# ivanalberico/End-To-End-Self-Supervised-SLAM

Measured on AMD Instinct MI355X. Metric: online refinement steps/sec @640x480, seq_len=60, higher is better.
Workload: dtype f32

## Files before the change

### end-to-end-self-supervised-slam_amd/csrc/conv.hip

```cpp
#include <cassert>
#include <type_traits>

#include "e2e_common.h"

typedef float f4v __attribute__((ext_vector_type(4)));
typedef float f16v __attribute__((ext_vector_type(16)));

#define CBK 16

enum { ACT_NONE = 0, ACT_RELU = 1, ACT_ELU = 2, ACT_DISP = 3 };

struct ConvArgs {
    const float* src0;
    const float* src1;
    const float* w;
    const float* scale;
    const float* shift;
    const float* res;
    float* out;
    int B, Hs, Ws;
    int Cin, C1, up;
    int Hd, Wd;
    int Ncols, ldw;
    int KH, KW, stride, pad, pad_mode;
// ... 1750 lines not shown
#pragma unroll
        for (int j = 0; j < PH; ++j) *(f4v*)&patch[(j * PW * 4 + tid) * 4] = preg[j];
        if (tid < PH * 8) *(f4v*)&patch[((epy * PW + epx) * 4 + pq) * 4] = preg[PH];
    };
    f4v acc[NA];
#pragma unroll
    for (int t = 0; t < NA; ++t) acc[t] = (f4v){0.f, 0.f, 0.f, 0.f};
    const float one = (l16 == 0) ? 1.f : 0.f;
    const float* bp = patch + (wave * PW + kq) * 16 + l16;
    auto sweep = [&](unsigned zn) {
        float bv[9];
#pragma unroll
        for (int t = 0; t < 9; ++t) bv[t] = bp[((t / 3) * PW + (t % 3)) * 16];
#pragma unroll
        for (int ks = 0; ks < TW / 4; ++ks) {
            float bn[9];
#pragma unroll
            for (int t = 0; t < 9; ++t) bn[t] = ks + 1 < TW / 4 ? bp[((t / 3) * PW + (t % 3)) * 16 + (ks + 1) * 64] : 0.f;
#pragma unroll
            for (int t = 0; t < 9; ++t)
#pragma unroll
                for (int mt = 0; mt < MT; ++mt) acc[mt * 10 + t] = __builtin_amdgcn_mfma_f32_16x16x4f32(areg[ks][mt], bv[t], acc[mt * 10 + t], 0, 0, 0);
            if constexpr (BIAS) {
#pragma unroll
                for (int mt = 0; mt < MT; ++mt) acc[mt * 10 + 9] = __builtin_amdgcn_mfma_f32_16x16x4f32(areg[ks][mt], one, acc[mt * 10 + 9], 0, 0, 0);
            }
#pragma unroll
            for (int mt = 0; mt < MT; ++mt)
                areg[ks][mt] = __builtin_bit_cast(float, __builtin_amdgcn_raw_buffer_load_b32(rz, zn + (unsigned)(ks * 4 * CO + mt * 16) * 4u, 0, 0));
#pragma unroll
            for (int t = 0; t < 9; ++t) bv[t] = bn[t];
            __builtin_amdgcn_sched_barrier(0);
        }
    };
    if (ntl > 0) {
        load_dz((unsigned)(tx0 * TW * CO) * 4u + zl);
        load_patch(tx0 * TW);
        store_patch();
    }
    __syncthreads();
    for (int tx = 0; tx < ntl; ++tx) {
        const bool more = tx + 1 < ntl;
        const int xn = (tx0 + tx + 1) * TW;
        const unsigned zn = more ? (unsigned)(xn * CO) * 4u + zl : OOB;
        if (more) load_patch(xn);
        sweep(zn);
        __syncthreads();
        if (more) {
            store_patch();
            __syncthreads();
        }
    }
    float* red = smem;
    const int64_t sid = ((int64_t)b * gridDim.y + blockIdx.y) * a.nxg + blockIdx.x;
    float* slab = a.slabs + sid * CO * a.npad;
    const int kconv = 9 * a.Cin, cg0 = hf * 16;
#pragma unroll
    for (int mt = 0; mt < MT; ++mt) {
        if (mt > 0) __syncthreads();
        if (wave >= 2) {
#pragma unroll
            for (int t = 0; t < 10; ++t)
#pragma unroll
                for (int i = 0; i < 4; ++i) red[((wave - 2) * 40 + t * 4 + i) * 64 + lane] = acc[mt * 10 + t][i];
        }
        __syncthreads();
        if (wave < 2) {
#pragma unroll
            for (int t = 0; t < 10; ++t)
#pragma unroll
                for (int i = 0; i < 4; ++i) acc[mt * 10 + t][i] += red[(wave * 40 + t * 4 + i) * 64 + lane];
        }
        __syncthreads();
        if (wave == 1) {
#pragma unroll
            for (int t = 0; t < 10; ++t)
#pragma unroll
                for (int i = 0; i < 4; ++i) red[(t * 4 + i) * 64 + lane] = acc[mt * 10 + t][i];
        }
        __syncthreads();
        if (wave == 0) {
#pragma unroll
            for (int t = 0; t < 10; ++t)
#pragma unroll
                for (int i = 0; i < 4; ++i) {
                    const float v = acc[mt * 10 + t][i] + red[(t * 4 + i) * 64 + lane];
                    const int co = mt * 16 + 4 * kq + i;
                    if (t < 9) slab[co * a.npad + t * a.Cin + cg0 + l16] = v;
                    else if (BIAS && l16 == 0) slab[co * a.npad + kconv] = v;
                }
        }
    }
}

template <int MT>
__global__ __launch_bounds__(256) __attribute__((amdgpu_waves_per_eu(MT == 1 ? 4 : 2))) void k_wgrad3x3_thin_regs(ThinWgradArgs a) {
    __shared__ float smem[6 * 66 * 16];
    if (a.has_bias && blockIdx.z % (a.Cin >> 4) == 0) wgrad3x3_thin_regs_body<MT, true>(a, smem);
    else wgrad3x3_thin_regs_body<MT, false>(a, smem);
}

struct StemWgradArgs {
    const float* dz;
    const float* src;
    float* slabs;
    int B, Hs, Ws, Hd, Wd, tiles_x, nxg;
    float in_sub, in_mul;
};

__global__ __launch_bounds__(256) void k_wgrad7x7_stem(StemWgradArgs a) {
    constexpr int TH = 4, TW = 32, PH = 2 * TH + 6, PW = 2 * TW + 5, ROW = 208, NPAD = 148;
    __shared__ float patch[PH * ROW];
    __shared__ float dzs[TH * TW * 64];
    const int tid = threadIdx.x, lane = tid & 63, wave = tid >> 6, l16 = lane & 15, kq = lane >> 4;
    const int y0 = blockIdx.y * TH, b = blockIdx.z;
    int offn[10];
#pragma unroll
    for (int nt = 0; nt < 10; ++nt) {
        const int k = 16 * nt + l16;
        offn[nt] = k + (k / 21) * (ROW - 21) + 48 * kq;
    }
    f4v acc[10];
#pragma unroll
    for (int nt = 0; nt < 10; ++nt) acc[nt] = (f4v){0.f, 0.f, 0.f, 0.f};
    const float* sb = a.src + (int64_t)b * a.Hs * a.Ws * 3;
    const float* zb = a.dz + (int64_t)b * a.Hd * a.Wd * 64;
    for (int tx = 0; tx < a.tiles_x; ++tx) {
        const int x0 = (blockIdx.x * a.tiles_x + tx) * TW;
        if (x0 >= a.Wd) break;
        __syncthreads();
        for (int idx = tid; idx < PH * ROW; idx += 256) {
            const int py = idx / ROW, e = idx - py * ROW;
            const int Y = 2 * y0 - 3 + py, X = 2 * x0 - 3 + e / 3;
            const bool ok = e < 3 * PW && Y >= 0 && Y < a.Hs && X >= 0 && X < a.Ws;
            patch[idx] = ok ? (sb[((int64_t)Y * a.Ws + X) * 3 + (e - (e / 3) * 3)] - a.in_sub) * a.in_mul : 0.f;
        }
        for (int idx = tid; idx < TH * TW * 16; idx += 256) {
            const int q = idx & 15, pix = idx >> 4;
            const int r = pix / TW, x = pix - r * TW;
            const bool ok = y0 + r < a.Hd && x0 + x < a.Wd;
            *(f4v*)&dzs[pix * 64 + q * 4] = ok ? *(const f4v*)(zb + ((int64_t)(y0 + r) * a.Wd + x0 + x) * 64 + q * 4) : (f4v){0.f, 0.f, 0.f, 0.f};
        }
        __syncthreads();
#pragma unroll 1
        for (int r = 0; r < TH; ++r) {
            const float* ap = dzs + (r * TW + 8 * kq) * 64 + 16 * wave + l16;
            const float* bp = patch + 2 * r * ROW;
#pragma unroll 2
            for (int ks = 0; ks < TW / 4; ++ks) {
                const float av = ap[ks * 64];
#pragma unroll
                for (int nt = 0; nt < 10; ++nt) acc[nt] = __builtin_amdgcn_mfma_f32_16x16x4f32(av, bp[offn[nt] + ks * 6], acc[nt], 0, 0, 0);
            }
        }
    }
    float* slab = a.slabs + (((int64_t)b * gridDim.y + blockIdx.y) * a.nxg + blockIdx.x) * 64 * NPAD;
#pragma unroll
    for (int nt = 0; nt < 10; ++nt)
#pragma unroll
        for (int i = 0; i < 4; ++i) {
            const int n = 16 * nt + l16;
            if (n < 147) slab[(16 * wave + 4 * kq + i) * NPAD + n] = acc[nt][i];
        }
}

struct TapWgradArgs {
    const float* dz;
    const float* src0;
    const float* src1;
    float* slabs;
    int B, H, W, Cin, C1, up, Cout, reflect, has_bias, Mpad, Npad;
    int ptx, pty;
    int nchunks, cps;
};

#define TAP_NT 192
template <bool BIAS>
__global__ __launch_bounds__(TAP_NT) void k_wgrad3x3_taps(TapWgradArgs a) {
    __shared__ float dzs[64 * 32];
    __shared__ float xs[100 * 32];
    const int tid = threadIdx.x, lane = tid & 63, wave = tid >> 6, kh_ = lane >> 5, l32 = lane & 31;
    const int ci0 = blockIdx.x * 32, co0 = blockIdx.y * 32;
    const bool first = ci0 < a.C1;
    const int sh = first ? (a.up >> 1) : 0, Cs = first ? a.C1 : a.Cin - a.C1, cs0 = first ? ci0 : ci0 - a.C1;
    const int Hs = a.H >> sh, Ws = a.W >> sh;
    const float* sbase = first ? a.src0 : a.src1;
    const int c_begin = blockIdx.z * a.cps, c_end = min(c_begin + a.cps, a.nchunks);
    const bool want_bias = BIAS && blockIdx.x == 0 && wave == 0;
    f16v acc[3], accb;
#pragma unroll
    for (int t = 0; t < 3; ++t)
#pragma unroll
        for (int r = 0; r < 16; ++r) acc[t][r] = 0.f;
#pragma unroll
    for (int r = 0; r < 16; ++r) accb[r] = 0.f;
    const float one = (l32 == 0) ? 1.f : 0.f;
    f4v rz[3], rx[5];
    auto load_chunk = [&](int g) {
        const int b = g / (a.pty * a.ptx), rem = g - b * (a.pty * a.ptx), py = rem / a.ptx, px = rem - py * a.ptx;
        const int y0 = py * 8, x0 = px * 8;
        const float* zb = a.dz + (int64_t)b * a.H * a.W * a.Cout + co0;
        const float* sb = sbase + (int64_t)b * Hs * Ws * Cs + cs0;
#pragma unroll
        for (int i = 0; i < 3; ++i) {
            const int f = tid + TAP_NT * i, pix = f >> 3, q = f & 7, y = y0 + (pix >> 3), x = x0 + (pix & 7);
            const bool ok = f < 512 && y < a.H && x < a.W;
            rz[i] = ok ? *(const f4v*)(zb + ((int64_t)y * a.W + x) * a.Cout + q * 4) : (f4v){0.f, 0.f, 0.f, 0.f};
        }
#pragma unroll
        for (int i = 0; i < 5; ++i) {
            const int f = tid + TAP_NT * i;
            f4v v = {0.f, 0.f, 0.f, 0.f};
            if (f < 800) {
                const int pix = f >> 3, q = f & 7;
                int y = y0 - 1 + pix / 10, x = x0 - 1 + pix % 10;
                bool ok = true;
                if (a.reflect) {
                    y = min(max(reflect1(y, a.H), 0), a.H - 1);
                    x = min(max(reflect1(x, a.W), 0), a.W - 1);
                } else {
                    ok = y >= 0 && y < a.H && x >= 0 && x < a.W;
                }
                if (ok) v = *(const f4v*)(sb + ((int64_t)(y >> sh) * Ws + (x >> sh)) * Cs + q * 4);
            }
            rx[i] = v;
        }
    };
    auto store_chunk = [&]() {
#pragma unroll
        for (int i = 0; i < 3; ++i) {
            const int f = tid + TAP_NT * i;
            if (f < 512) *(f4v*)&dzs[f * 4] = rz[i];
        }
#pragma unroll
        for (int i = 0; i < 5; ++i) {
            const int f = tid + TAP_NT * i;
            if (f < 800) *(f4v*)&xs[f * 4] = rx[i];
        }
    };
    if (c_begin < c_end) load_chunk(c_begin);
    const float* ap = dzs + kh_ * 32 + l32;
    const float* bp = xs + (kh_ + wave * 10) * 32 + l32;
    for (int c = c_begin; c < c_end; ++c) {
        __syncthreads();
        store_chunk();
        __syncthreads();
        if (c + 1 < c_end) load_chunk(c + 1);
        constexpr int QB = 4, NQ = 32 / QB;
        float av[2][QB], bv[2][QB][3];
        auto read_q = [&](int set, int qt) {
#pragma unroll
            for (int j = 0; j < QB; ++j) {
                const int ks = QB * qt + j, q0 = (ks >> 2) * 10 + 2 * (ks & 3);
                av[set][j] = ap[2 * ks * 32];
#pragma unroll
                for (int t = 0; t < 3; ++t) bv[set][j][t] = bp[(q0 + t) * 32];
            }
        };
        auto pin_q = [&](int set) {
#pragma unroll
            for (int j = 0; j < QB; ++j) {
                asm volatile("" : "+v"(av[set][j]));
#pragma unroll
                for (int t = 0; t < 3; ++t) asm volatile("" : "+v"(bv[set][j][t]));
            }
        };
        read_q(0, 0);
#pragma unroll
        for (int qt = 0; qt < NQ; ++qt) {
            if (qt + 1 < NQ) read_q((qt + 1) & 1, qt + 1);
            __builtin_amdgcn_sched_barrier(0);
            pin_q(qt & 1);
            __builtin_amdgcn_sched_barrier(0);
#pragma unroll
            for (int j = 0; j < QB; ++j) {
#pragma unroll
                for (int t = 0; t < 3; ++t) acc[t] = __builtin_amdgcn_mfma_f32_32x32x2f32(av[qt & 1][j], bv[qt & 1][j][t], acc[t], 0, 0, 0);
                if (BIAS && want_bias) accb = __builtin_amdgcn_mfma_f32_32x32x2f32(av[qt & 1][j], one, accb, 0, 0, 0);
            }
            __builtin_amdgcn_sched_barrier(0);
        }
    }
    float* slab = a.slabs + (int64_t)blockIdx.z * a.Mpad * a.Npad;
#pragma unroll
    for (int t = 0; t < 3; ++t)
#pragma unroll
        for (int r = 0; r < 16; ++r) {
            const int m = co0 + (r & 3) + 8 * (r >> 2) + 4 * kh_;
            slab[(int64_t)m * a.Npad + (wave * 3 + t) * a.Cin + ci0 + l32] = acc[t][r];
        }
    if (BIAS && want_bias && l32 == 0) {
#pragma unroll
        for (int r = 0; r < 16; ++r) slab[(int64_t)(co0 + (r & 3) + 8 * (r >> 2) + 4 * kh_) * a.Npad + 9 * a.Cin] = accb[r];
    }
}

template <int ZL, int NW>
__device__ __forceinline__ void wgrad_reduce_group(const float* __restrict__ slabs, int S, int Mpad, int Npad, int Cout, int Cin, int KH, int KW, int has_bias,
                                                   float* __restrict__ dw, float* __restrict__ dbias, int accumulate, const float* __restrict__ scale,
                                                   int64_t base, int e, int w, f4v (*part)[64]) {
    const int Kconv = KH * KW * Cin, Ng = Kconv + (has_bias ? 1 : 0);
    const int nq = (Ng + 3) / 4;
    const int64_t totalq = (int64_t)Cout * nq;
    const int64_t slab_q = (int64_t)Mpad * Npad / 4;
    const f4v zero = {0.f, 0.f, 0.f, 0.f};
    const int64_t q = base + e;
// ... 1036 lines not shown
#define HEAD_PARTS 2048
int e2e_head_fwd(const float* x, const float* w, const float* bias, float* y, int B, int H, int W, int Cin, int act, void* stream) {
    E2E_REQUIRE(x && w && y && B > 0 && H >= 2 && W >= 2 && Cin == HC, E2E_ERR_ARG, "e2e_head_fwd: bad argument (the head takes %d channels)", HC);
    hipLaunchKernelGGL(k_head_fwd, dim3(egrid((int64_t)B * H * W * 4)), dim3(256), 0, (hipStream_t)stream, x, w, bias, y, B, H, W, act);
    E2E_LAUNCH_CHECK("e2e_head_fwd");
    return E2E_OK;
}
int64_t e2e_head_workspace_floats(void) { return (int64_t)HEAD_PARTS * (9 * HC + 1); }
int e2e_head_bwd_act(const float* dz, const float* x, const float* w, float* dx, float* dw, float* dbias, float* workspace, int B, int H,
                     int W, int Cin, int in_act, void* stream) {
    E2E_REQUIRE(dz && x && w && workspace && B > 0 && H >= 2 && W >= 2 && Cin == HC && in_act >= 0 && in_act <= 2, E2E_ERR_ARG, "e2e_head_bwd: bad argument");
    E2E_REQUIRE((int64_t)B * H * W * HC < (1ll << 31), E2E_ERR_ARG, "e2e_head_bwd: activation too large for 32-bit element offsets");
    hipStream_t st = (hipStream_t)stream;
    const char* ev = getenv("E2E_HEAD_BWD_FUSED");
    if (dx && dw && !(ev && ev[0] == '0')) {
        hipLaunchKernelGGL(k_head_bwd_fused, dim3(HEAD_PARTS), dim3(256), 0, st, dz, x, w, dx, workspace, B, H, W, in_act);
        hipLaunchKernelGGL(k_head_wreduce, dim3(9 * HC + 1), dim3(256), 0, st, workspace, HEAD_PARTS, dw, dbias);
        E2E_LAUNCH_CHECK("e2e_head_bwd");
        return E2E_OK;
    }
    if (dx) hipLaunchKernelGGL(k_head_bwd_data, dim3(egrid((int64_t)B * H * W * 4)), dim3(256), 0, st, dz, w, dx, B, H, W, x, in_act);
    if (dw) {
        hipLaunchKernelGGL(k_head_bwd_weight, dim3(HEAD_PARTS), dim3(256), 0, st, dz, x, workspace, B, H, W);
        hipLaunchKernelGGL(k_head_wreduce, dim3(9 * HC + 1), dim3(256), 0, st, workspace, HEAD_PARTS, dw, dbias);
    }
    E2E_LAUNCH_CHECK("e2e_head_bwd");
    return E2E_OK;
}

int e2e_head_bwd(const float* dz, const float* x, const float* w, float* dx, float* dw, float* dbias, float* workspace, int B, int H,
                 int W, int Cin, void* stream) {
    return e2e_head_bwd_act(dz, x, w, dx, dw, dbias, workspace, B, H, W, Cin, 0, stream);
}

enum WgradPath { WP_STEM, WP_THIN, WP_TAPS, WP_GEMM16, WP_GEMM_LEAN, WP_GEMM, WP_COUNT };
struct WgradPlan { WgradPath path; bool open; int64_t S; int Mpad, Npad, tm, tn, nxg, ny, tiles_x, ptx, pty, nchunks, cps; };
#define TAP_TARGET 640
static WgradPlan wgrad_plan(WgradPath path, const ConvGeom& g, int has_bias, bool tuned, int wg_target) {
    const int B = g.B, Ho = g.Ho, Wo = g.Wo, Cin = g.Cin, Cout = g.Cout, KH = g.KH, KW = g.KW;
    WgradPlan p{path};
    if (path == WP_STEM) {
        if (tuned || !(KH == 7 && KW == 7 && Cin == 3 && Cout == 64)) return p;
        p.nxg = ((Wo + 31) / 32 + 1) / 2; p.ny = (Ho + 3) / 4;
        p.S = (int64_t)B * p.ny * p.nxg; p.Mpad = 64; p.Npad = 148;
    } else if (path == WP_THIN) {
        if (tuned || !(KH == 3 && KW == 3 && ((Cout == 16 && (Cin == 16 || Cin == 32)) || (Cout == 32 && Cin == 96)))) return p;
        const int txt = (Wo + 63) / 64;
        p.ny = (Ho + 3) / 4;
        const int64_t total = (int64_t)B * p.ny * txt * (Cin / 16);
        p.tiles_x = 1;
        while (total / p.tiles_x > 1400 && p.tiles_x < txt) ++p.tiles_x;
        p.nxg = (txt + p.tiles_x - 1) / p.tiles_x;
        p.S = (int64_t)B * p.ny * p.nxg; p.Mpad = Cout; p.Npad = (9 * Cin + (has_bias ? 1 : 0) + 3) / 4 * 4;
    } else if (path == WP_TAPS) {
        if (tuned || !(KH == 3 && KW == 3 && Cin % 32 == 0 && Cout % 32 == 0)) return p;
        p.ptx = (Wo + 7) / 8; p.pty = (Ho + 7) / 8;
        p.nchunks = B * p.ptx * p.pty;
        const int tiles = (Cin / 32) * (Cout / 32);
        int S = (TAP_TARGET + tiles - 1) / tiles;
        if (S > p.nchunks) S = p.nchunks;
        if (S < 1) S = 1;
        p.cps = (p.nchunks + S - 1) / S;
        p.S = (p.nchunks + p.cps - 1) / p.cps; p.Mpad = Cout; p.Npad = (9 * Cin + (has_bias ? 1 : 0) + 3) / 4 * 4;
    } else {
        const bool use16 = path == WP_GEMM16;
        if (use16 && Cout != 16) return p;
        const int Ng = KH * KW * Cin + (has_bias ? 1 : 0);
        p.tm = Cout <= 32 ? 32 : 64; p.tn = Cout <= 32 ? 128 : 64;
        if (use16) { p.tm = 16; p.tn = 160; }
        p.Mpad = (Cout + p.tm - 1) / p.tm * p.tm; p.Npad = (Ng + p.tn - 1) / p.tn * p.tn;
        const int64_t P = (int64_t)B * Ho * Wo;
        const int64_t tiles = (int64_t)(p.Mpad / p.tm) * (p.Npad / p.tn);
        const int target = use16 ? wg_target * 3 / 4 : wg_target;
        int64_t S = (target + tiles - 1) / tiles;
        const int64_t maxS = (P + 255) / 256;
        if (S > maxS) S = maxS;
        if (S < 1) S = 1;
        p.S = S;
    }
    p.open = true;
    return p;
}

static int64_t wgrad_workspace_floats(const ConvGeom& g, int has_bias, bool tuned, int wg_target) {
    int64_t n = 0;
    for (int i = 0; i < WP_COUNT; ++i) {
        const WgradPlan p = wgrad_plan((WgradPath)i, g, has_bias, tuned, wg_target);
        if (p.open && p.S * p.Mpad * p.Npad > n) n = p.S * p.Mpad * p.Npad;
    }
    return n;
}

static WgradPlan wgrad_choose(const ConvGeom& g, int has_bias, bool has_src1, bool tuned, int wg_target) {
    const int Hs = g.Hs, Ws = g.Ws, Cin = g.Cin, Cout = g.Cout, Ho = g.Ho, Wo = g.Wo, stride = g.stride, pad = g.pad, pad_mode = g.pad_mode, C1 = g.C1, up = g.up;
    const int vec = (Cin % 4 == 0 && C1 % 4 == 0) ? 4 : 1;
    const int64_t P = (int64_t)g.B * Ho * Wo;
    auto plan = [&](WgradPath w) { return wgrad_plan(w, g, has_bias, tuned, wg_target); };
    const bool lean = vec == 4 && Cout % 4 == 0 && Wo >= 8 && (int64_t)g.B * Hs * Ws * Cin * 4 < (1ll << 31) && P * Cout * 4 < (1ll << 31) && P < (1ll << 24);
    WgradPlan p{WP_GEMM};
    if (stride == 2 && pad == 3 && pad_mode == 0 && C1 == Cin && up == 1 && !has_bias && Ho == (Hs + 6 - 7) / 2 + 1 && Wo == (Ws + 6 - 7) / 2 + 1 &&
        (p = plan(WP_STEM)).open)
        return p;
    if (lean && stride == 1 && pad == 1 && pad_mode == 1 && C1 % 16 == 0 && Ho == Hs && Wo == Ws && (C1 == Cin || has_src1) && Hs % up == 0 && Ws % up == 0 &&
        (p = plan(WP_THIN)).open)
        return p;
    if (vec == 4 && stride == 1 && pad == 1 && Ho == Hs && Wo == Ws && (up == 1 || up == 2) && Hs % up == 0 && Ws % up == 0 && (C1 == Cin || (has_src1 && C1 % 32 == 0)) &&
        getenv("E2E_WGRAD_TAPS") != nullptr && getenv("E2E_WGRAD_TAPS")[0] == '1' && (p = plan(WP_TAPS)).open)
        return p;
    return lean && (p = plan(WP_GEMM16)).open ? p : plan(lean ? WP_GEMM_LEAN : WP_GEMM);
}

int64_t e2e_conv2d_wgrad_workspace_floats(int B, int Ho, int Wo, int Cin, int Cout, int KH, int KW, int has_bias) {
    GEOM_WGRAD_QUERY(g);
    return wgrad_workspace_floats(g, has_bias, false, WGRAD_TARGET);
}

struct WgradOut { float* dw; float* dbias; const float* out_scale; int accumulate; e2e_wgrad_reduce_desc* defer; };

static void wgrad_reduce(const WgradArgs& a, const WgradOut& o, int S, int Mpad, int Npad, int zl, hipStream_t st) {
    if (o.defer) {
        *o.defer = e2e_wgrad_reduce_desc{a.slabs, o.dw, o.dbias, o.out_scale, S, Mpad, Npad, a.Cout, a.Cin, a.KH, a.KW, a.has_bias, o.accumulate, zl, 0};
        return;
    }
    const int64_t tq = (int64_t)a.Cout * ((a.Ngemm + 3) / 4);
    if (zl == 8)
        hipLaunchKernelGGL((k_wgrad_reduce<8>), dim3(egrid(tq * 4)), dim3(512), 0, st, a.slabs, S, Mpad, Npad, a.Cout, a.Cin, a.KH, a.KW, a.has_bias, o.dw,
                           o.dbias, o.accumulate, o.out_scale);
    else
        hipLaunchKernelGGL((k_wgrad_reduce<2>), dim3(egrid(tq * 4)), dim3(128), 0, st, a.slabs, S, Mpad, Npad, a.Cout, a.Cin, a.KH, a.KW, a.has_bias, o.dw,
                           o.dbias, o.accumulate, o.out_scale);
}

enum WgradKernel { WK_DONE, WK_GEMM16, WK_GEMM4_32, WK_GEMM4_64, WK_GEMM_32, WK_GEMM_64 };
struct WgradLaunch { WgradKernel k; dim3 g; int Sz; };

static int wgrad_setup(const WgradIn& in, const ConvGeom& g, int wg_target, const WgradOut& o, hipStream_t st, WgradArgs& a, WgradLaunch& L, bool dry = false) {
    const int B = g.B, Cin = g.Cin, Cout = g.Cout, Ho = g.Ho, Wo = g.Wo;
    const bool tuned = wg_target != 0;
    if (!tuned) wg_target = WGRAD_TARGET;
    L = WgradLaunch{WK_DONE, dim3(1), 0};
    E2E_REQUIRE(in.dz && in.src0 && o.dw && in.workspace && B > 0 && Cin > 0 && Cout > 0, E2E_ERR_ARG, "e2e_conv2d_bwd_weight: bad argument");
    const int vec = (Cin % 4 == 0 && g.C1 % 4 == 0) ? 4 : 1;
    E2E_REQUIRE(vec == 4 || (g.C1 == Cin && g.up == 1 && g.pad_mode == 0), E2E_ERR_ARG, "e2e_conv2d_bwd_weight: scalar path takes one full-resolution zero-padded source");
    a = WgradArgs{};
    a.dz = in.dz; a.src0 = in.src0; a.src1 = in.src1; a.slabs = in.workspace;
    a.B = B; a.Hs = g.Hs; a.Ws = g.Ws; a.Cin = Cin; a.C1 = g.C1; a.up = g.up; a.Ho = Ho; a.Wo = Wo; a.Cout = Cout;
    a.KH = g.KH; a.KW = g.KW; a.stride = g.stride; a.pad = g.pad; a.pad_mode = g.pad_mode; a.has_bias = o.dbias ? 1 : 0;
    a.Ngemm = g.KH * g.KW * Cin + a.has_bias;
    const WgradPlan p = wgrad_choose(g, a.has_bias, in.src1 != nullptr, tuned, wg_target);
    const int S = (int)p.S;
    if (dry && (p.path == WP_STEM || p.path == WP_THIN || p.path == WP_TAPS)) return E2E_OK;
    if (p.path == WP_STEM) {
        StemWgradArgs ta{in.dz, in.src0, in.workspace, B, g.Hs, g.Ws, Ho, Wo, 2, p.nxg, g.in_sub, g.in_mul};
        hipLaunchKernelGGL(k_wgrad7x7_stem, dim3(p.nxg, p.ny, B), dim3(256), 0, st, ta);
    } else if (p.path == WP_THIN) {
        ThinWgradArgs ta{in.dz, in.src0, in.src1, in.workspace, B, Ho, Wo, Cin, g.C1, g.up, p.Npad, a.has_bias, p.tiles_x, p.nxg};
        const dim3 tg((unsigned)p.nxg, (unsigned)p.ny, (unsigned)(B * (Cin / 16)));
        const char* ev = getenv("E2E_THIN_WGRAD_REGS");
        const bool regs = !(ev && ev[0] == '0') && (int64_t)Wo * Cout * 4 < (1ll << 31);
        if (regs && Cout == 32) hipLaunchKernelGGL((k_wgrad3x3_thin_regs<2>), tg, dim3(256), 0, st, ta);
        else if (regs) hipLaunchKernelGGL((k_wgrad3x3_thin_regs<1>), tg, dim3(256), 0, st, ta);
        else if (Cout == 32) hipLaunchKernelGGL((k_wgrad3x3_thin<2>), tg, dim3(256), 0, st, ta);
        else hipLaunchKernelGGL((k_wgrad3x3_thin<1>), tg, dim3(256), 0, st, ta);
    } else if (p.path == WP_TAPS) {
        TapWgradArgs ta{in.dz, in.src0, in.src1, in.workspace, B, Ho, Wo, Cin, g.C1, g.up, Cout, g.pad_mode == 1 ? 1 : 0, a.has_bias,
                        p.Mpad, p.Npad, p.ptx, p.pty, p.nchunks, p.cps};
        const dim3 tg((unsigned)(Cin / 32), (unsigned)(Cout / 32), (unsigned)S);
        if (a.has_bias) hipLaunchKernelGGL(k_wgrad3x3_taps<true>, tg, dim3(TAP_NT), 0, st, ta);
        else hipLaunchKernelGGL(k_wgrad3x3_taps<false>, tg, dim3(TAP_NT), 0, st, ta);
    }
    if (p.path == WP_STEM || p.path == WP_THIN || p.path == WP_TAPS) {
        wgrad_reduce(a, o, S, p.Mpad, p.Npad, (p.path == WP_TAPS && S < 8) ? 2 : 8, st);
        return E2E_OK;
    }
    const bool use16 = p.path == WP_GEMM16, lean = p.path != WP_GEMM;
    a.Mpad = p.Mpad; a.Npad = p.Npad;
    a.in_sub = g.in_sub; a.in_mul = g.in_mul; a.vec = vec;
    const int64_t P = (int64_t)B * Ho * Wo;
    const int cbp = lean ? 32 : CBK;
    a.pix_per_slice = ((P + p.S - 1) / p.S + cbp - 1) / cbp * cbp;
    L.Sz = (int)((P + a.pix_per_slice - 1) / a.pix_per_slice);
    L.g = dim3((unsigned)(a.Npad / p.tn), (unsigned)(a.Mpad / p.tm), (unsigned)L.Sz);
    L.k = use16 ? WK_GEMM16 : lean ? (p.tm == 32 ? WK_GEMM4_32 : WK_GEMM4_64) : (p.tm == 32 ? WK_GEMM_32 : WK_GEMM_64);
    return E2E_OK;
}

static void wgrad_launch_gemm(const WgradArgs& a, const WgradLaunch& L, hipStream_t st) {
    const dim3 g = L.g;
    const bool two = a.src1 != nullptr;
    if (L.k == WK_GEMM16) hipLaunchKernelGGL((k_wgrad_gemm16<10, 32>), g, dim3(256), 0, st, a);
    else if (L.k == WK_GEMM4_32 && two) hipLaunchKernelGGL((k_wgrad_gemm4<1, 4, 32, true>), g, dim3(256), 0, st, a);
    else if (L.k == WK_GEMM4_32) hipLaunchKernelGGL((k_wgrad_gemm4<1, 4, 32, false>), g, dim3(256), 0, st, a);
    else if (L.k == WK_GEMM4_64 && two) hipLaunchKernelGGL((k_wgrad_gemm4<2, 2, 32, true>), g, dim3(256), 0, st, a);
    else if (L.k == WK_GEMM4_64) hipLaunchKernelGGL((k_wgrad_gemm4<2, 2, 32, false>), g, dim3(256), 0, st, a);
    else if (L.k == WK_GEMM_32 && a.vec == 4) hipLaunchKernelGGL((k_wgrad_gemm<1, 4, 4>), g, dim3(256), 0, st, a);
    else if (L.k == WK_GEMM_32) hipLaunchKernelGGL((k_wgrad_gemm<1, 4, 1>), g, dim3(256), 0, st, a);
    else if (L.k == WK_GEMM_64 && a.vec == 4) hipLaunchKernelGGL((k_wgrad_gemm<2, 2, 4>), g, dim3(256), 0, st, a);
    else if (L.k == WK_GEMM_64) hipLaunchKernelGGL((k_wgrad_gemm<2, 2, 1>), g, dim3(256), 0, st, a);
}

static int bwd_weight_impl(const WgradIn& in, const ConvGeom& g, const WgradOut& o, void* stream, int wg_target = 0) {
    const hipStream_t st = (hipStream_t)stream;
    WgradArgs a;
    WgradLaunch L;
    const int rc = wgrad_setup(in, g, wg_target, o, st, a, L);
    if (rc != E2E_OK) return rc;
    if (L.k != WK_DONE) {
        wgrad_launch_gemm(a, L, st);
        wgrad_reduce(a, o, L.Sz, a.Mpad, a.Npad, L.Sz >= 8 ? 8 : 2, st);
    }
    E2E_LAUNCH_CHECK("e2e_conv2d_bwd_weight");
    return E2E_OK;
}

int e2e_conv2d_bwd_weight(const float* dz, const float* src0, const float* src1, int C1, int up, float* dw, float* dbias,
                          float* workspace, int B, int Hs, int Ws, int Cin, int Cout, int Ho, int Wo, int KH, int KW, int stride,
                          int pad, int pad_mode, int accumulate, float in_sub, float in_mul, void* stream) {
    GEOM_BWD_WEIGHT(g);
    return bwd_weight_impl(WgradIn{dz, src0, src1, workspace}, g, WgradOut{dw, dbias, nullptr, accumulate, nullptr}, stream);
}

int e2e_conv2d_bwd_weight_scaled(const float* da, const float* out_scale, const float* src0, const float* src1, int C1, int up, float* dw,
                                 float* dbias, float* workspace, int B, int Hs, int Ws, int Cin, int Cout, int Ho, int Wo, int KH, int KW,
                                 int stride, int pad, int pad_mode, int accumulate, float in_sub, float in_mul, void* stream) {
    GEOM_BWD_WEIGHT(g);
    return bwd_weight_impl(WgradIn{da, src0, src1, workspace}, g, WgradOut{dw, dbias, out_scale, accumulate, nullptr}, stream);
}

int e2e_conv2d_bwd_weight_scaled_deferred(const float* da, const float* out_scale, const float* src0, const float* src1, int C1, int up, float* dw,
                                          float* dbias, float* workspace, int B, int Hs, int Ws, int Cin, int Cout, int Ho, int Wo, int KH, int KW,
                                          int stride, int pad, int pad_mode, int accumulate, float in_sub, float in_mul,
                                          e2e_wgrad_reduce_desc* desc_out, void* stream) {
    E2E_REQUIRE(desc_out, E2E_ERR_ARG, "e2e_conv2d_bwd_weight_scaled_deferred: desc_out is NULL");
    GEOM_BWD_WEIGHT(g);
    return bwd_weight_impl(WgradIn{da, src0, src1, workspace}, g, WgradOut{dw, dbias, out_scale, accumulate, desc_out}, stream);
}

struct PairOps {
    const float *da, *w_bwd; int ld_bwd; float* dxp; int accumulate; const float* x_in; int in_act; const float* pre_add; float* workspace;
    const float *out_scale, *src0, *src1; float *dw, *dbias, *workspace_w; int accumulate_w; e2e_wgrad_reduce_desc* desc_out;
};
struct PairCarry { const e2e_wgrad_reduce_desc* descs; int n; long long first, items; int place; };
#ifndef CARRY_WGS
#define CARRY_WGS 2048
#endif

struct PairPlan { ConvArgs ad; bool data_done; WgradArgs aw; WgradLaunch lw; GemmLaunch pd; bool paired, d14; };

static int bwd_pair_plan(const PairOps& q, const ConvGeom& g, const WgradOut& o, hipStream_t st, PairPlan& P, bool dry) {
    int rc = bwd_data_setup(BwdDataOps{q.da, q.w_bwd, q.ld_bwd, q.dxp, q.accumulate, q.x_in, q.in_act, q.pre_add}, g, GemmCfg{0, 0, 0}, st, P.ad, P.data_done, dry);
    if (rc != E2E_OK) return rc;
    rc = wgrad_setup(WgradIn{q.da, q.src0, q.src1, q.workspace_w}, g, 0, o, st, P.aw, P.lw, dry);
    if (rc != E2E_OK) return rc;
    P.pd = GemmLaunch{};
    if (!P.data_done) P.pd = plan_gemm<true>(P.ad, 4, q.workspace, GemmCfg{0, 0, 0});
    P.d14 = P.pd.c.bm == 32 && P.pd.c.bn == 128;
    const bool d22 = P.pd.c.bm == 64 && P.pd.c.bn == 64;
    P.paired = !P.data_done && P.pd.kind == GK_TILE && P.pd.cb == 32 && (P.d14 || d22) && P.lw.k == WK_GEMM4_64;
    return E2E_OK;
}

static int wgrad_reduce_range(const e2e_wgrad_reduce_desc* descs_dev, int n, long long first_item, long long items, hipStream_t st) {
    hipLaunchKernelGGL(k_wgrad_reduce_batched, dim3((unsigned)(items < 4096 ? items : 4096)), dim3(512), 0, st, descs_dev, n, first_item, items);
    return E2E_OK;
}

static int bwd_pair_impl(const PairOps& q, const ConvGeom& g, int wgrad_first, const PairCarry& cy, const char* who, void* stream) {
    E2E_REQUIRE(q.desc_out, E2E_ERR_ARG, "%s: desc_out is NULL", who);
    E2E_REQUIRE(cy.items >= 0 && cy.first >= 0 && (cy.items == 0 || (cy.descs && cy.n > 0)) && cy.place >= 0 && cy.place <= 2, E2E_ERR_ARG,
                "%s: bad carry range", who);
    const hipStream_t st = (hipStream_t)stream;
    const WgradOut o{q.dw, q.dbias, q.out_scale, q.accumulate_w, q.desc_out};
    PairPlan P;
    const int rc = bwd_pair_plan(q, g, o, st, P, false);
    if (rc != E2E_OK) return rc;
    ConvArgs& ad = P.ad;
    const WgradArgs& aw = P.aw;
    const WgradLaunch& lw = P.lw;
    if (P.paired) {
        PairGrid pg;
        pg.dgx = P.pd.g.x; pg.dgy = P.pd.g.y; pg.dgz = P.pd.g.z;
        pg.wgx = lw.g.x; pg.wgy = lw.g.y; pg.wgz = lw.g.z;
        const unsigned nd = pg.dgx * pg.dgy * pg.dgz, nw = pg.wgx * pg.wgy * pg.wgz;
        pg.wgrad_first = wgrad_first ? 1 : 0;
        pg.first = ((wgrad_first ? nw : nd) + 7u) / 8u * 8u;
        const unsigned second = wgrad_first ? nd : nw;
        CarryArgs ca{cy.descs, cy.n, (unsigned)(cy.items < CARRY_WGS ? cy.items : CARRY_WGS), cy.first, cy.items};
        pg.cbeg = 0xffffffffu; pg.cpad = 0;
        if (ca.wgs) {
            pg.cbeg = cy.place == 0 ? pg.first + second : cy.place == 1 ? pg.first : 0u;
            pg.cpad = cy.place == 0 ? ca.wgs : (ca.wgs + 7u) / 8u * 8u;
        }
        const dim3 grid(pg.first + second + pg.cpad);
        const bool two = aw.src1 != nullptr;
        if (P.d14) {
            if (two) hipLaunchKernelGGL((k_conv_bwd_pair<1, 4, true>), grid, dim3(256), 0, st, ad, aw, pg, ca);
            else hipLaunchKernelGGL((k_conv_bwd_pair<1, 4, false>), grid, dim3(256), 0, st, ad, aw, pg, ca);
        } else {
            if (two) hipLaunchKernelGGL((k_conv_bwd_pair<2, 2, true>), grid, dim3(256), 0, st, ad, aw, pg, ca);
            else hipLaunchKernelGGL((k_conv_bwd_pair<2, 2, false>), grid, dim3(256), 0, st, ad, aw, pg, ca);
        }
    } else {
        if (!P.data_done) launch_gemm_main<true>(ad, P.pd, q.workspace, st);
        if (lw.k != WK_DONE) wgrad_launch_gemm(aw, lw, st);
    }
    if (!P.data_done) launch_gemm_tail(ad, P.pd, st);
    if (lw.k != WK_DONE) wgrad_reduce(aw, o, lw.Sz, aw.Mpad, aw.Npad, lw.Sz >= 8 ? 8 : 2, st);
// ... 83 lines not shown
```

Baseline: 226.5.

## Add register-pipelined 7x7 stem weight-gradient kernel with buffer loads

Adds a variant of the 7x7 stem weight-gradient kernel that keeps the output-gradient operand in registers and loads it directly from global memory with buffer loads, instead of staging it through shared memory. The next tile's input patch and gradients are prefetched into registers while the current tile's MFMAs run, which is meant to hide global-memory latency and remove one shared-memory round trip and its barriers. It is enabled by default, with an environment variable to turn it off and a size guard for 32-bit buffer offsets. The cost is higher register pressure, with occupancy pinned via waves_per_eu, and more complex scheduling.

```diff
diff --git a/end-to-end-self-supervised-slam_amd/csrc/conv.hip b/end-to-end-self-supervised-slam_amd/csrc/conv.hip
--- a/end-to-end-self-supervised-slam_amd/csrc/conv.hip
+++ b/end-to-end-self-supervised-slam_amd/csrc/conv.hip
@@ -1926,6 +1926,111 @@
 #pragma unroll
                 for (int nt = 0; nt < 10; ++nt) acc[nt] = __builtin_amdgcn_mfma_f32_16x16x4f32(av, bp[offn[nt] + ks * 6], acc[nt], 0, 0, 0);
             }
+        }
+    }
+    float* slab = a.slabs + (((int64_t)b * gridDim.y + blockIdx.y) * a.nxg + blockIdx.x) * 64 * NPAD;
+#pragma unroll
+    for (int nt = 0; nt < 10; ++nt)
+#pragma unroll
+        for (int i = 0; i < 4; ++i) {
+            const int n = 16 * nt + l16;
+            if (n < 147) slab[(16 * wave + 4 * kq + i) * NPAD + n] = acc[nt][i];
+        }
+}
+
+__global__ __launch_bounds__(256) __attribute__((amdgpu_waves_per_eu(3))) void k_wgrad7x7_stem_regs(StemWgradArgs a) {
+    constexpr int TH = 4, TW = 32, PH = 2 * TH + 6, PW = 2 * TW + 5, ROW = 208, NPAD = 148;
+    constexpr int ITEMS = PH * PW, NL = (ITEMS + 255) / 256;
+    constexpr unsigned OOB = 0x80000000u;
+    typedef float f2v __attribute__((ext_vector_type(2)));
+    __shared__ float patch[PH * ROW];
+    const int tid = threadIdx.x, lane = tid & 63, wave = __builtin_amdgcn_readfirstlane(tid >> 6), l16 = lane & 15, kq = lane >> 4;
+    const int y0 = blockIdx.y * TH, b = blockIdx.z;
+    const int tx0 = blockIdx.x * a.tiles_x;
+    const int ntl = min(a.tiles_x, (a.Wd + TW - 1) / TW - tx0);
+    int offn[10];
+#pragma unroll
+    for (int nt = 0; nt < 10; ++nt) {
+        const int k = 16 * nt + l16;
+        offn[nt] = k + (k / 21) * (ROW - 21) + 48 * kq;
+    }
+    f4v acc[10];
+#pragma unroll
+    for (int nt = 0; nt < 10; ++nt) acc[nt] = (f4v){0.f, 0.f, 0.f, 0.f};
+    __amdgpu_buffer_rsrc_t rz[TH];
+#pragma unroll
+    for (int r = 0; r < TH; ++r)
+        rz[r] = __builtin_amdgcn_make_buffer_rsrc((void*)(a.dz + ((int64_t)b * a.Hd + min(y0 + r, a.Hd - 1)) * a.Wd * 64), 0,
+                                                  y0 + r < a.Hd ? a.Wd * 64 * 4 : 0, 0x00020000);
+    const unsigned zl = (unsigned)(8 * kq * 64 + 16 * wave + l16) * 4u;
+    float areg[TH][TW / 4];
+    auto load_dz = [&](unsigned zo) {
+#pragma unroll
+        for (int r = 0; r < TH; ++r)
+#pragma unroll
+            for (int ks = 0; ks < TW / 4; ++ks) areg[r][ks] = __builtin_bit_cast(float, __builtin_amdgcn_raw_buffer_load_b32(rz[r], zo + (unsigned)(ks * 64) * 4u, 0, 0));
+    };
+    const __amdgpu_buffer_rsrc_t rs = __builtin_amdgcn_make_buffer_rsrc((void*)a.src, 0, a.B * a.Hs * a.Ws * 3 * 4, 0x00020000);
+    float preg[NL][3];
+    auto item_ok = [&](int k, int x0, int& py, int& px, int& Y, int& X) {
+        const int idx = tid + 256 * k;
+        py = idx / PW; px = idx - py * PW;
+        Y = 2 * y0 - 3 + py; X = 2 * x0 - 3 + px;
+        return idx < ITEMS && Y >= 0 && Y < a.Hs && X >= 0 && X < a.Ws;
+    };
+    auto load_patch = [&](int x0) {
+#pragma unroll
+        for (int k = 0; k < NL; ++k) {
+            int py, px, Y, X;
+            const bool ok = item_ok(k, x0, py, px, Y, X);
+            const unsigned off = ok ? (unsigned)((b * a.Hs + Y) * a.Ws + X) * 12u : OOB;
+            const f2v rg = __builtin_bit_cast(f2v, __builtin_amdgcn_raw_buffer_load_b64(rs, off, 0, 0));
+            preg[k][0] = rg[0]; preg[k][1] = rg[1];
+            preg[k][2] = __builtin_bit_cast(float, __builtin_amdgcn_raw_buffer_load_b32(rs, off + 8u, 0, 0));
+        }
+    };
+    auto store_patch = [&](int x0) {
+#pragma unroll
+        for (int k = 0; k < NL; ++k) {
+            int py, px, Y, X;
+            const bool ok = item_ok(k, x0, py, px, Y, X);
+            if (tid + 256 * k >= ITEMS) continue;
+#pragma unroll
+            for (int c = 0; c < 3; ++c)
+                patch[py * ROW + 3 * px + c] = ok ? (preg[k][c] - a.in_sub) * a.in_mul : 0.f;
+        }
+    };
+    auto sweep = [&](unsigned zn) {
+#pragma unroll
+        for (int r = 0; r < TH; ++r) {
+            const float* bp = patch + 2 * r * ROW;
+#pragma unroll
+            for (int ks = 0; ks < TW / 4; ++ks) {
+                float bv[10];
+#pragma unroll
+                for (int nt = 0; nt < 10; ++nt) bv[nt] = bp[offn[nt] + ks * 6];
+#pragma unroll
+                for (int nt = 0; nt < 10; ++nt) acc[nt] = __builtin_amdgcn_mfma_f32_16x16x4f32(areg[r][ks], bv[nt], acc[nt], 0, 0, 0);
+                areg[r][ks] = __builtin_bit_cast(float, __builtin_amdgcn_raw_buffer_load_b32(rz[r], zn + (unsigned)(ks * 64) * 4u, 0, 0));
+                __builtin_amdgcn_sched_barrier(0);
+            }
+        }
+    };
+    if (ntl > 0) {
+        load_dz((unsigned)(tx0 * TW * 64) * 4u + zl);
+        load_patch(tx0 * TW);
+        store_patch(tx0 * TW);
+    }
+    __syncthreads();
+    for (int tx = 0; tx < ntl; ++tx) {
+        const bool more = tx + 1 < ntl;
+        const int xn = (tx0 + tx + 1) * TW;
+        if (more) load_patch(xn);
+        sweep(more ? (unsigned)(xn * 64) * 4u + zl : OOB);
+        __syncthreads();
+        if (more) {
+            store_patch(xn);
+            __syncthreads();
         }
     }
     float* slab = a.slabs + (((int64_t)b * gridDim.y + blockIdx.y) * a.nxg + blockIdx.x) * 64 * NPAD;
@@ -3268,7 +3373,10 @@
     if (dry && (p.path == WP_STEM || p.path == WP_THIN || p.path == WP_TAPS)) return E2E_OK;
     if (p.path == WP_STEM) {
         StemWgradArgs ta{in.dz, in.src0, in.workspace, B, g.Hs, g.Ws, Ho, Wo, 2, p.nxg, g.in_sub, g.in_mul};
-        hipLaunchKernelGGL(k_wgrad7x7_stem, dim3(p.nxg, p.ny, B), dim3(256), 0, st, ta);
+        const char* ev = getenv("E2E_STEM_WGRAD_REGS");
+        const bool regs = !(ev && ev[0] == '0') && (int64_t)Wo * 64 * 4 < (1ll << 31) && (int64_t)B * g.Hs * g.Ws * 12 < (1ll << 31);
+        if (regs) hipLaunchKernelGGL(k_wgrad7x7_stem_regs, dim3(p.nxg, p.ny, B), dim3(256), 0, st, ta);
+        else hipLaunchKernelGGL(k_wgrad7x7_stem, dim3(p.nxg, p.ny, B), dim3(256), 0, st, ta);
     } else if (p.path == WP_THIN) {
         ThinWgradArgs ta{in.dz, in.src0, in.src1, in.workspace, B, Ho, Wo, Cin, g.C1, g.up, p.Npad, a.has_bias, p.tiles_x, p.nxg};
         const dim3 tg((unsigned)p.nxg, (unsigned)p.ny, (unsigned)(B * (Cin / 16)));
```

New measurement: 227.0, median of 6. No clear change (+0.2%).
